# BenWibking/amrVolumeRenderer

Hardware: AMD Instinct MI355X
Metric: Mray-samples/s (2048x2048 render of 512^3-base 3-level AMR) (higher is better)
Workload: dtype f32 march / f64 cell fetch+transform; 1 GPU; config4_amr3_512: 176 boxes of 128^3 (2.95 GB f64), 3 AMR levels, field=smooth, 2048x2048, antialiasing=1, box_transparency=0.97, default jet map, 1 view(s); ownership=level_pairs, runs_total=1, frame_driver=C++ (avr_renderer: 3 HIP streams), march_workgroups_per_cu=0, classification=every frame, samples_per_frame=759136367, camera=static (the frame plan is made once)

## Files before the change

amrvolumerenderer_amd/csrc/avr_kernels.hip:

```cpp
#include <hip/hip_runtime.h>

#include <algorithm>
#include <cmath>
#include <cstdint>
#include <type_traits>

#include "avr_internal.h"
#include "avr_device.h"

namespace avr {

namespace {

constexpr int kBlockThreads = 256;
#ifndef AVR_MARCH_GROUP
#define AVR_MARCH_GROUP 8
#endif

#define AVR_INF __builtin_huge_valf()

struct Layer5 {
  float r, g, b, a, d;
};

// ... 13 lines not shown
  const float t = 1.0f - front.a;
  Layer5 out;
  out.r = front.r + back.r * t;
  out.g = front.g + back.g * t;
  out.b = front.b + back.b * t;
  out.a = front.a + back.a * t;
  out.d = (bottom.d < top.d) ? bottom.d : top.d;
  return out;
}

struct Ray {
  float ox, oy, oz;
  float dx, dy, dz;
};

__device__ __forceinline__ Ray make_ray(int px, int py, const FrameConsts& fc) {
  const float ndc_x = (static_cast<float>(px) + 0.5f) * fc.inv_width * 2.0f - 1.0f;
  const float ndc_y = (static_cast<float>(py) + 0.5f) * fc.inv_height * 2.0f - 1.0f;
  const float plane_x = ndc_x * fc.tan_half_fov * fc.aspect;
  const float plane_y = ndc_y * fc.tan_half_fov;
  Ray ray;
  ray.dx = fc.fwd[0] + plane_x * fc.right[0] + plane_y * fc.up[0];
  ray.dy = fc.fwd[1] + plane_x * fc.right[1] + plane_y * fc.up[1];
  ray.dz = fc.fwd[2] + plane_x * fc.right[2] + plane_y * fc.up[2];
  const float len_sq = ray.dx * ray.dx + ray.dy * ray.dy + ray.dz * ray.dz;
  const float len = (len_sq > 0.0f) ? (1.0f / (1.0f / sqrtf(len_sq))) : 0.0f;
  if (len > 0.0f) {
    const float inv = 1.0f / len;
    ray.dx *= inv;
    ray.dy *= inv;
    ray.dz *= inv;
  }
  ray.ox = fc.eye[0];
  ray.oy = fc.eye[1];
  ray.oz = fc.eye[2];
  return ray;
}

__device__ __forceinline__ void slab_axis(float origin, float direction, float inv_dir,
                                          float min_val, float max_val, float& tmin,
                                          float& tmax) {
  if (fabsf(direction) < 1e-8f) {
    if (origin < min_val || origin > max_val) {
      tmin = AVR_INF;
      tmax = -AVR_INF;
    }
    return;
  }
  float t1 = (min_val - origin) * inv_dir;
  float t2 = (max_val - origin) * inv_dir;
  if (t1 > t2) {
    const float tmp = t1;
    t1 = t2;
    t2 = tmp;
  }
  tmin = (tmin > t1) ? tmin : t1;
  tmax = (tmax < t2) ? tmax : t2;
}

__device__ __forceinline__ uint32_t bricklet_offset(int i, int j, int k, uint32_t y_pitch,
                                                    uint32_t x_pitch) {
  const uint32_t ui = static_cast<uint32_t>(i), uj = static_cast<uint32_t>(j),
                 uk = static_cast<uint32_t>(k);
  uint32_t offset;
  asm("v_lshl_add_u32 %0, %1, 3, %2" : "=v"(offset) : "v"(uj), "v"(ui));
  asm("v_lshl_add_u32 %0, %1, 5, %0" : "+v"(offset) : "v"(uk));
  asm("v_mad_u32_u24 %0, %1, %2, %0" : "+v"(offset) : "v"(uj >> 2), "s"(y_pitch));
  asm("v_mad_u32_u24 %0, %1, %2, %0" : "+v"(offset) : "v"(ui >> 3), "s"(x_pitch));
  return offset;
}

template <bool LINEAR>
__device__ __forceinline__ uint32_t cell_address(int i, int j, int k, uint32_t y_pitch,
                                                 uint32_t x_pitch) {
  if constexpr (LINEAR) {
    return (static_cast<uint32_t>(i) + static_cast<uint32_t>(j) * y_pitch +
            static_cast<uint32_t>(k) * x_pitch) << 3;
  } else {
    return bricklet_offset(i, j, k, y_pitch, x_pitch);
  }
}

typedef float float_pair __attribute__((ext_vector_type(2)));

template <int MODE, bool CLAMP, bool STATS, bool LINEAR = false>
__device__ __forceinline__ uint32_t offset_from_quotients(const BoxDev& box, uint32_t row_pitch,
                                                          uint32_t plane_pitch, float qx, float qy,
                                                          float qz, float fx, float fy, float fz,
                                                          unsigned& near_hits) {
  int i = static_cast<int>(qx);
  int j = static_cast<int>(qy);
  int k = static_cast<int>(qz);
  if (CLAMP) {
    i = (i > box.nx - 1) ? box.nx - 1 : i;
    j = (j > box.ny - 1) ? box.ny - 1 : j;
    k = (k > box.nz - 1) ? box.nz - 1 : k;
  }
  if (MODE == kReciprocal) {
    const float ex = fabsf(qx - rintf(qx));
    const float ey = fabsf(qy - rintf(qy));
    const float ez = fabsf(qz - rintf(qz));
    if (fminf(fminf(ex, ey), ez) <= box.near_tol) {
      if (STATS) ++near_hits;
      int ei = static_cast<int>(floorf(fx / box.dx));
      int ej = static_cast<int>(floorf(fy / box.dy));
      int ek = static_cast<int>(floorf(fz / box.dz));
      i = (ei < 0) ? 0 : ((ei >= box.nx) ? box.nx - 1 : ei);
      j = (ej < 0) ? 0 : ((ej >= box.ny) ? box.ny - 1 : ej);
      k = (ek < 0) ? 0 : ((ek >= box.nz) ? box.nz - 1 : ek);
    }
  }
  return cell_address<LINEAR>(i, j, k, row_pitch, plane_pitch);
}

template <int MODE, bool STATS, bool LINEAR = false>
__device__ __forceinline__ uint32_t cell_offset(const BoxDev& box, uint32_t row_pitch,
                                                uint32_t plane_pitch, float fx, float fy,
                                                float fz, unsigned& near_hits) {
  if (MODE == kExactDivide) {
    int ei = static_cast<int>(floorf(fx / box.dx));
    int ej = static_cast<int>(floorf(fy / box.dy));
    int ek = static_cast<int>(floorf(fz / box.dz));
    ei = (ei < 0) ? 0 : ((ei >= box.nx) ? box.nx - 1 : ei);
    ej = (ej < 0) ? 0 : ((ej >= box.ny) ? box.ny - 1 : ej);
    ek = (ek < 0) ? 0 : ((ek >= box.nz) ? box.nz - 1 : ek);
    return cell_address<LINEAR>(ei, ej, ek, row_pitch, plane_pitch);
  }
  return offset_from_quotients<MODE, true, STATS, LINEAR>(box, row_pitch, plane_pitch, fx * box.inv_dx,
                                                  fy * box.inv_dy, fz * box.inv_dz, fx, fy, fz,
                                                  near_hits);
}

struct ColumnSum {
  double sum;
  unsigned count;
};
template <FrameKind KIND> struct MarchOf { using Result = Layer5; using RayArg = const Ray&; };
template <> struct MarchOf<FrameKind::kMaxIntensity> { using Result = int; using RayArg = const Ray; };
template <> struct MarchOf<FrameKind::kProjection> { using Result = ColumnSum; using RayArg = const Ray; };

template <bool STATS, int MODE, FrameKind KIND = FrameKind::kVolume>
__device__ __forceinline__ typename MarchOf<KIND>::Result
march_box(const BoxDev& box, const FrameConsts& fc,
                                            const uint8_t* __restrict__ classified,
                                            const float4* __restrict__ table,
                                            typename MarchOf<KIND>::RayArg ray,
                                            float tmin, float tmax, unsigned& fetches,
                                            unsigned& near_hits) {
  constexpr bool is_max = KIND == FrameKind::kMaxIntensity, is_sum = KIND == FrameKind::kProjection;
  const float min_x = box.minc[0], min_y = box.minc[1], min_z = box.minc[2];
  const float max_x = box.maxc[0], max_y = box.maxc[1], max_z = box.maxc[2];
  const float step = box.sample_dist;
  const uint8_t __attribute__((address_space(1)))* cells =
      (const uint8_t __attribute__((address_space(1)))*)(classified + box.cls_offset);
  const uint32_t bricks_z = static_cast<uint32_t>(box.nz + kBrickZ - 1) >> 2;
  const uint32_t bricks_y = static_cast<uint32_t>(box.ny + kBrickY - 1) >> 2;
  const uint32_t row_pitch = is_sum ? static_cast<uint32_t>(box.jstride)
                                 : bricks_z * kBrickBytes - 32u;
  const uint32_t plane_pitch = is_sum ? static_cast<uint32_t>(box.kstride)
                                   : bricks_y * bricks_z * kBrickBytes - 8u;
  [[maybe_unused]] const uint8_t __attribute__((address_space(1)))* values =
      (const uint8_t __attribute__((address_space(1)))*)(box.cells);

  float distance = tmin + box.mesh_eps;
  if (distance < 0.0f) distance = box.mesh_eps;

  float acc_r = 0.0f, acc_g = 0.0f, acc_b = 0.0f, acc_a = 0.0f;
  [[maybe_unused]] int best = -1;
  [[maybe_unused]] double sum = 0.0;
  [[maybe_unused]] unsigned count = 0u;

#define AVR_INSIDE(x, y, z) \
  (!((x) < min_x || (x) > max_x || (y) < min_y || (y) > max_y || (z) < min_z || (z) > max_z))
#define AVR_VALUE(offset) \
  (*reinterpret_cast<const double __attribute__((address_space(1)))*>(values + (offset)))
#define AVR_ADD(value)                                  \
  do {                                                  \
    const bool finite_ = __builtin_isfinite(value);     \
    sum += finite_ ? (value) : 0.0;                     \
    count += finite_ ? 1u : 0u;                         \
  } while (0)
#define AVR_ACCUMULATE(sample)                          \
  do {                                                  \
    const float alpha_ = (sample).w * (1.0f - acc_a);   \
    acc_r += (sample).x * alpha_;                       \
    acc_g += (sample).y * alpha_;                       \
    acc_b += (sample).z * alpha_;                       \
    acc_a += alpha_;                                    \
  } while (0)

  const float safe_end = tmax - step;
  bool interior = false;
  if (distance < safe_end) {
    const float ax = ray.ox + ray.dx * distance, ay = ray.oy + ray.dy * distance,
                az = ray.oz + ray.dz * distance;
    const float bx = ray.ox + ray.dx * safe_end, by = ray.oy + ray.dy * safe_end,
                bz = ray.oz + ray.dz * safe_end;
    interior = AVR_INSIDE(ax, ay, az) && AVR_INSIDE(bx, by, bz);
    if (MODE != kExactDivide) {
      const int ia = static_cast<int>((ax - min_x) * box.inv_dx), ib = static_cast<int>((bx - min_x) * box.inv_dx);
      const int ja = static_cast<int>((ay - min_y) * box.inv_dy), jb = static_cast<int>((by - min_y) * box.inv_dy);
      const int ka = static_cast<int>((az - min_z) * box.inv_dz), kb = static_cast<int>((bz - min_z) * box.inv_dz);
      interior = interior && ia < box.nx && ib < box.nx && ja < box.ny && jb < box.ny &&
                 ka < box.nz && kb < box.nz;
    }
  }
  if (interior) {
    const float inv_x = box.inv_dx, inv_y = box.inv_dy, inv_z = box.inv_dz;
    const float_pair ix2 = {inv_x, inv_x}, iy2 = {inv_y, inv_y}, iz2 = {inv_z, inv_z};
    float_pair nx2 = {box.nmin_inv[0], box.nmin_inv[0]}, ny2 = {box.nmin_inv[1], box.nmin_inv[1]},
               nz2 = {box.nmin_inv[2], box.nmin_inv[2]};
    if (MODE == kPow2Multiply) asm volatile("" : "+v"(nx2), "+v"(ny2), "+v"(nz2));
#if AVR_MARCH_GROUP > 4
    if (MODE == kPow2Multiply || MODE == kReciprocal) {
      constexpr int kDeep = AVR_MARCH_GROUP;
      static_assert(kDeep % 2 == 0, "the positions are computed two at a time");
      for (;;) {
        float d[kDeep];
        d[0] = distance;
#pragma unroll
        for (int i = 1; i < kDeep; ++i) d[i] = d[i - 1] + step;
        if (!(d[kDeep - 1] < safe_end)) break;
        uint32_t off[kDeep];
#pragma unroll
        for (int pair = 0; pair < kDeep / 2; ++pair) {
          const float_pair dd = {d[2 * pair], d[2 * pair + 1]};
          if (MODE == kPow2Multiply) {
            const float_pair qx = __builtin_elementwise_fma(ray.ox + ray.dx * dd, ix2, nx2);
            const float_pair qy = __builtin_elementwise_fma(ray.oy + ray.dy * dd, iy2, ny2);
            const float_pair qz = __builtin_elementwise_fma(ray.oz + ray.dz * dd, iz2, nz2);
            off[2 * pair] = cell_address<is_sum>(static_cast<int>(qx.x), static_cast<int>(qy.x),
                                            static_cast<int>(qz.x), row_pitch, plane_pitch);
            off[2 * pair + 1] = cell_address<is_sum>(static_cast<int>(qx.y), static_cast<int>(qy.y),
                                                static_cast<int>(qz.y), row_pitch, plane_pitch);
          } else {
            const float_pair fx = (ray.ox + ray.dx * dd) - min_x;
            const float_pair fy = (ray.oy + ray.dy * dd) - min_y;
            const float_pair fz = (ray.oz + ray.dz * dd) - min_z;
            const float_pair qx = fx * inv_x, qy = fy * inv_y, qz = fz * inv_z;
            off[2 * pair] = offset_from_quotients<MODE, false, STATS, is_sum>(
                box, row_pitch, plane_pitch, qx.x, qy.x, qz.x, fx.x, fy.x, fz.x, near_hits);
            off[2 * pair + 1] = offset_from_quotients<MODE, false, STATS, is_sum>(
                box, row_pitch, plane_pitch, qx.y, qy.y, qz.y, fx.y, fy.y, fz.y, near_hits);
          }
        }
        if constexpr (is_sum) {
          double v[kDeep];
#pragma unroll
          for (int i = 0; i < kDeep; ++i) v[i] = AVR_VALUE(off[i]);
#pragma unroll
          for (int i = 0; i < kDeep; ++i) AVR_ADD(v[i]);
          distance = d[kDeep - 1] + step;
          if (STATS) fetches += static_cast<unsigned>(kDeep);
          continue;
        }
        int idx[kDeep];
#pragma unroll
        for (int i = 0; i < kDeep; ++i) idx[i] = cells[off[i]];
        if constexpr (is_max) {
#pragma unroll
          for (int i = 0; i < kDeep; ++i) best = (idx[i] > best) ? idx[i] : best;
          distance = d[kDeep - 1] + step;
          if (STATS) fetches += static_cast<unsigned>(kDeep);
          continue;
        }
        float4 sample[kDeep];
#pragma unroll
        for (int i = 0; i < kDeep; ++i) sample[i] = table[idx[i]];
        float_pair rg = {acc_r, acc_g}, ba = {acc_b, acc_a};
#pragma unroll
        for (int i = 0; i < kDeep; ++i) {
          const float w_ = sample[i].w * (1.0f - ba.y);
          const float_pair color_ = {sample[i].x, sample[i].y};
          const float_pair zw_ = {sample[i].z * w_, w_};
          float_pair weighted_;
          asm("v_pk_mul_f32 %0, %1, %2 op_sel:[0,1] op_sel_hi:[1,1]"
              : "=v"(weighted_)
              : "v"(color_), "v"(zw_));
          ba = ba + zw_;
          rg = rg + weighted_;
          asm volatile("" : "+v"(rg));
        }
        if (__builtin_amdgcn_ballot_w64(ba.y >= 1.0f) == 0) {
          acc_r = rg.x;
          acc_g = rg.y;
          acc_b = ba.x;
          acc_a = ba.y;
          distance = d[kDeep - 1] + step;
          if (STATS) fetches += static_cast<unsigned>(kDeep);
        } else {
          unsigned taken = 0u;
          float next = distance;
#pragma unroll
          for (int i = 0; i < kDeep; ++i) {
            const bool running_ = acc_a < 1.0f;
            const float alpha_ = sample[i].w * (1.0f - acc_a);
            const float r_ = acc_r + sample[i].x * alpha_;
            const float g_ = acc_g + sample[i].y * alpha_;
            const float b_ = acc_b + sample[i].z * alpha_;
            const float a_ = acc_a + alpha_;
            acc_r = running_ ? r_ : acc_r;
            acc_g = running_ ? g_ : acc_g;
            acc_b = running_ ? b_ : acc_b;
            acc_a = running_ ? a_ : acc_a;
            next = running_ ? (d[i] + step) : next;
            taken += running_ ? 1u : 0u;
          }
          distance = next;
          if (STATS) fetches += taken;
          if (!(acc_a < 1.0f)) break;
        }
      }
    }
#endif
    for (;;) {
      const float d1 = distance;
      const float d2 = d1 + step;
      const float d3 = d2 + step;
      const float d4 = d3 + step;
      if (!(d4 < safe_end)) break;
      uint32_t off1, off2, off3, off4;
      if (MODE == kExactDivide) {
        off1 = cell_offset<MODE, STATS, is_sum>(box, row_pitch, plane_pitch,
                                        (ray.ox + ray.dx * d1) - min_x,
                                        (ray.oy + ray.dy * d1) - min_y,
                                        (ray.oz + ray.dz * d1) - min_z, near_hits);
        off2 = cell_offset<MODE, STATS, is_sum>(box, row_pitch, plane_pitch,
                                        (ray.ox + ray.dx * d2) - min_x,
                                        (ray.oy + ray.dy * d2) - min_y,
                                        (ray.oz + ray.dz * d2) - min_z, near_hits);
        off3 = cell_offset<MODE, STATS, is_sum>(box, row_pitch, plane_pitch,
                                        (ray.ox + ray.dx * d3) - min_x,
                                        (ray.oy + ray.dy * d3) - min_y,
                                        (ray.oz + ray.dz * d3) - min_z, near_hits);
        off4 = cell_offset<MODE, STATS, is_sum>(box, row_pitch, plane_pitch,
                                        (ray.ox + ray.dx * d4) - min_x,
                                        (ray.oy + ray.dy * d4) - min_y,
                                        (ray.oz + ray.dz * d4) - min_z, near_hits);
      } else if (MODE == kPow2Multiply) {
        const float_pair d12 = {d1, d2}, d34 = {d3, d4};
        const float_pair qx12 = __builtin_elementwise_fma(ray.ox + ray.dx * d12, ix2, nx2);
        const float_pair qy12 = __builtin_elementwise_fma(ray.oy + ray.dy * d12, iy2, ny2);
        const float_pair qz12 = __builtin_elementwise_fma(ray.oz + ray.dz * d12, iz2, nz2);
        const float_pair qx34 = __builtin_elementwise_fma(ray.ox + ray.dx * d34, ix2, nx2);
        const float_pair qy34 = __builtin_elementwise_fma(ray.oy + ray.dy * d34, iy2, ny2);
        const float_pair qz34 = __builtin_elementwise_fma(ray.oz + ray.dz * d34, iz2, nz2);
        off1 = cell_address<is_sum>(static_cast<int>(qx12.x), static_cast<int>(qy12.x),
                               static_cast<int>(qz12.x), row_pitch, plane_pitch);
        off2 = cell_address<is_sum>(static_cast<int>(qx12.y), static_cast<int>(qy12.y),
                               static_cast<int>(qz12.y), row_pitch, plane_pitch);
        off3 = cell_address<is_sum>(static_cast<int>(qx34.x), static_cast<int>(qy34.x),
                               static_cast<int>(qz34.x), row_pitch, plane_pitch);
        off4 = cell_address<is_sum>(static_cast<int>(qx34.y), static_cast<int>(qy34.y),
                               static_cast<int>(qz34.y), row_pitch, plane_pitch);
      } else {
        const float_pair d12 = {d1, d2}, d34 = {d3, d4};
        const float_pair fx12 = (ray.ox + ray.dx * d12) - min_x, fx34 = (ray.ox + ray.dx * d34) - min_x;
        const float_pair fy12 = (ray.oy + ray.dy * d12) - min_y, fy34 = (ray.oy + ray.dy * d34) - min_y;
        const float_pair fz12 = (ray.oz + ray.dz * d12) - min_z, fz34 = (ray.oz + ray.dz * d34) - min_z;
        const float_pair qx12 = fx12 * inv_x, qx34 = fx34 * inv_x;
        const float_pair qy12 = fy12 * inv_y, qy34 = fy34 * inv_y;
        const float_pair qz12 = fz12 * inv_z, qz34 = fz34 * inv_z;
        off1 = offset_from_quotients<MODE, false, STATS, is_sum>(box, row_pitch, plane_pitch, qx12.x,
                                                         qy12.x, qz12.x, fx12.x, fy12.x, fz12.x,
                                                         near_hits);
        off2 = offset_from_quotients<MODE, false, STATS, is_sum>(box, row_pitch, plane_pitch, qx12.y,
                                                         qy12.y, qz12.y, fx12.y, fy12.y, fz12.y,
                                                         near_hits);
        off3 = offset_from_quotients<MODE, false, STATS, is_sum>(box, row_pitch, plane_pitch, qx34.x,
                                                         qy34.x, qz34.x, fx34.x, fy34.x, fz34.x,
                                                         near_hits);
        off4 = offset_from_quotients<MODE, false, STATS, is_sum>(box, row_pitch, plane_pitch, qx34.y,
                                                         qy34.y, qz34.y, fx34.y, fy34.y, fz34.y,
                                                         near_hits);
      }
      if constexpr (is_sum) {
        const double v1 = AVR_VALUE(off1);
        const double v2 = AVR_VALUE(off2);
        const double v3 = AVR_VALUE(off3);
        const double v4 = AVR_VALUE(off4);
        AVR_ADD(v1);
        AVR_ADD(v2);
        AVR_ADD(v3);
        AVR_ADD(v4);
        distance = d4 + step;
        if (STATS) fetches += 4u;
        continue;
      }
      const int idx1 = cells[off1];
      const int idx2 = cells[off2];
      const int idx3 = cells[off3];
      const int idx4 = cells[off4];
      if constexpr (is_max) {
        const int m12 = (idx1 > idx2) ? idx1 : idx2;
        const int m34 = (idx3 > idx4) ? idx3 : idx4;
        const int m = (m12 > m34) ? m12 : m34;
        best = (m > best) ? m : best;
        distance = d4 + step;
        if (STATS) fetches += 4u;
        continue;
      }
      const float4 s1 = table[idx1];
      const float4 s2 = table[idx2];
      const float4 s3 = table[idx3];
      const float4 s4 = table[idx4];
      float_pair rg = {acc_r, acc_g}, ba = {acc_b, acc_a};
#define AVR_STEP(sample)                                                          \
      {                                                                           \
        const float w_ = (sample).w * (1.0f - ba.y);                              \
        const float_pair color_ = {(sample).x, (sample).y};                       \
        const float_pair zw_ = {(sample).z * w_, w_};                             \
        float_pair weighted_;                                                     \
        asm("v_pk_mul_f32 %0, %1, %2 op_sel:[0,1] op_sel_hi:[1,1]"                \
            : "=v"(weighted_)                                                     \
            : "v"(color_), "v"(zw_));                                             \
        ba = ba + zw_;                                                            \
        rg = rg + weighted_;                                                      \
        asm volatile("" : "+v"(rg));                                              \
      }
      AVR_STEP(s1)
      AVR_STEP(s2)
      AVR_STEP(s3)
      AVR_STEP(s4)
#undef AVR_STEP
      if (__builtin_amdgcn_ballot_w64(ba.y >= 1.0f) == 0) {
        acc_r = rg.x;
        acc_g = rg.y;
        acc_b = ba.x;
        acc_a = ba.y;
// ... 11 lines not shown
          const float g_ = acc_g + (sample).y * alpha_;       \
          const float b_ = acc_b + (sample).z * alpha_;       \
          const float a_ = acc_a + alpha_;                    \
          acc_r = running_ ? r_ : acc_r;                      \
          acc_g = running_ ? g_ : acc_g;                      \
          acc_b = running_ ? b_ : acc_b;                      \
          acc_a = running_ ? a_ : acc_a;                      \
          next = running_ ? (following) : next;               \
          taken += running_ ? 1u : 0u;                        \
        }
        AVR_ACCUMULATE_IF_RUNNING(s2, d3)
        AVR_ACCUMULATE_IF_RUNNING(s3, d4)
        AVR_ACCUMULATE_IF_RUNNING(s4, d4 + step)
#undef AVR_ACCUMULATE_IF_RUNNING
        distance = next;
        if (STATS) fetches += taken;
        if (!(acc_a < 1.0f)) break;
      }
    }
  }

  float pos_x = ray.ox + ray.dx * distance;
  float pos_y = ray.oy + ray.dy * distance;
  float pos_z = ray.oz + ray.dz * distance;

  while (distance < tmax && (is_max || is_sum || acc_a < 1.0f)) {
    if (AVR_INSIDE(pos_x, pos_y, pos_z)) {
      const uint32_t offset = cell_offset<MODE, STATS, is_sum>(
          box, row_pitch, plane_pitch, pos_x - min_x, pos_y - min_y, pos_z - min_z, near_hits);
      if constexpr (is_sum) {
        const double v = AVR_VALUE(offset);
        if (STATS) ++fetches;
        AVR_ADD(v);
      } else {
      const int idx = cells[offset];
      if (STATS) ++fetches;
      if constexpr (is_max) {
        best = (idx > best) ? idx : best;
      } else {
        const float4 sample = table[idx];
        AVR_ACCUMULATE(sample);
      }
      }
    }
    distance += step;
    pos_x = ray.ox + ray.dx * distance;
    pos_y = ray.oy + ray.dy * distance;
    pos_z = ray.oz + ray.dz * distance;
  }
#undef AVR_INSIDE
#undef AVR_ACCUMULATE
#undef AVR_VALUE
#undef AVR_ADD

  if constexpr (is_sum) {
    return ColumnSum{sum, count};
  } else if constexpr (is_max) {
    return best;
  } else {
    acc_r = (acc_r > 1.0f) ? 1.0f : acc_r;
    acc_g = (acc_g > 1.0f) ? 1.0f : acc_g;
    acc_b = (acc_b > 1.0f) ? 1.0f : acc_b;
    acc_a = (acc_a > 1.0f) ? 1.0f : acc_a;
    Layer5 out;
    out.r = (acc_r < 0.0f) ? 0.0f : acc_r;
    out.g = (acc_g < 0.0f) ? 0.0f : acc_g;
    out.b = (acc_b < 0.0f) ? 0.0f : acc_b;
    out.a = (acc_a < 0.0f) ? 0.0f : acc_a;

    float depth = AVR_INF;
    if (acc_a > 0.0f) {
      const float ex = ray.ox + ray.dx * tmin;
      const float ey = ray.oy + ray.dy * tmin;
      const float ez = ray.oz + ray.dz * tmin;
      depth = (ex - fc.eye[0]) * fc.fwd[0] + (ey - fc.eye[1]) * fc.fwd[1] +
              (ez - fc.eye[2]) * fc.fwd[2];
    }
    if (!__builtin_isfinite(depth) || out.a <= 0.0f) depth = AVR_INF;
    out.d = depth;
    return out;
  }
}

template <bool STATS, int ONLY_MODE, bool SPEC, FrameKind KIND = FrameKind::kVolume>
__device__ __forceinline__ void
render_runs_body(
    const FrameConsts& fc, const BoxDev* __restrict__ boxes,
    const uint8_t* __restrict__ classified, const float* __restrict__ tables,
    const int n_tables, const int32_t* __restrict__ order, const int4* __restrict__ order_rects,
    const int32_t* __restrict__ run_end,
    const int n_runs, const int n_pieces, const RunRectDev* __restrict__ run_rects,
    const RunBlockDev* __restrict__ run_blocks, const RunSpanDev* __restrict__ run_spans,
    const int band_shift,
    const int tiles_x, const int tiles_y,
    const MarchItemDev* __restrict__ items, float* __restrict__ out,
    unsigned long long* samples_out, unsigned long long* counters,
    const int pos_begin, const int pos_end, const int resume,
    uint8_t* __restrict__ visible_out,
    const MarchSpecDev* __restrict__ spec) {
  constexpr bool is_max = KIND == FrameKind::kMaxIntensity, is_sum = KIND == FrameKind::kProjection;
  extern __shared__ float4 lds_tables[];
  if (SPEC && spec != nullptr) {
    const uint32_t* const gate = spec->gate;
    if (gate != nullptr) {
      if (*gate == 0) return;
      const uint8_t* const dirty = spec->dirty_blocks;
      if (dirty != nullptr && dirty[blockIdx.x] == 0) return;
    }
  }

  const unsigned b = blockIdx.x;
  const unsigned xcd = b % kXcds;
  const unsigned within = b / kXcds;
  const MarchItemDev item = items[(within / kSuperTileTiles) * kXcds + xcd];
  if (item.slot == kNoMarchItem) return;
  const unsigned seq = item.slot * kSuperTileTiles + (within % kSuperTileTiles);
  const int tile_x = static_cast<int>(compact_bits(seq));
  const int tile_y = static_cast<int>(compact_bits(seq >> 1));
  if (tile_x >= tiles_x || tile_y >= tiles_y) return;
  const int run = static_cast<int>(item.run);
  const RunRectDev rect = run_rects[run];
  if (rect.x1 < tile_x * kTile || rect.x0 > tile_x * kTile + kTile - 1 ||
      rect.y1 < tile_y * kTile || rect.y0 > tile_y * kTile + kTile - 1) {
    return;
  }

  if constexpr (!is_sum) {
  {
    const float4* src = reinterpret_cast<const float4*>(tables);
    const int total = n_tables * kTableSize;
    for (int e = threadIdx.x; e < total; e += kBlockThreads) lds_tables[e] = src[e];
  }
  __syncthreads();
  }

  const int wave = __builtin_amdgcn_readfirstlane(static_cast<int>(threadIdx.x) >> 6);
  const int lane = static_cast<int>(threadIdx.x) & 63;
  constexpr int kWaveW = 8, kWaveH = 8;
  const int wave_x0 = tile_x * kTile + (wave & 1) * 8;
  const int wave_y0 = tile_y * kTile + (wave >> 1) * 8;
  const int px = wave_x0 + (lane & 3) + ((lane >> 2) & 4);
  const int py = wave_y0 + ((lane >> 2) & 3) + ((lane >> 3) & 4);
  const bool live = (px < fc.width) && (py < fc.height);
  const int64_t n_pixels = static_cast<int64_t>(fc.width) * fc.height;
  const int64_t p = static_cast<int64_t>(py) * fc.width + px;

  const Ray ray = make_ray(px, py, fc);
  const float inv_dx = 1.0f / ray.dx;
  const float inv_dy = 1.0f / ray.dy;
  const float inv_dz = 1.0f / ray.dz;

  unsigned fetches = 0;
  unsigned near_hits = 0, mode_fetches[3] = {0u, 0u, 0u};
  {
    auto layer_pixel = [&]() -> float* {
      if (!(live && px >= rect.x0 && px <= rect.x1 && py >= rect.y0 && py <= rect.y1)) return nullptr;
      int64_t piece;
      int row = py;
      if (band_shift >= 0) {
        const unsigned band = static_cast<unsigned>(py) >> band_shift;
        const unsigned cycle = band / static_cast<unsigned>(n_pieces);
        piece = band - cycle * static_cast<unsigned>(n_pieces);
        row = static_cast<int>((cycle << band_shift) + (static_cast<unsigned>(py) & ((1u << band_shift) - 1u)));
      } else {
        const int64_t piece_size = n_pixels / n_pieces;
        piece = (piece_size > 0) ? (p / piece_size) : (n_pieces - 1);
        if (piece > n_pieces - 1) piece = n_pieces - 1;
      }
      const RunBlockDev block = run_blocks[static_cast<int64_t>(run) * n_pieces + piece];
      if (block.span_base >= 0) {
        const RunSpanDev span = run_spans[block.span_base + (row - block.first_row)];
        if (px < static_cast<int>(span.x0) || px > static_cast<int>(span.x1)) return nullptr;
        return out + block.offset + span.rel + static_cast<int64_t>(px - static_cast<int>(span.x0)) * 5;
      }
      return out + block.offset +
             (static_cast<int64_t>(row - block.first_row) * (rect.x1 - rect.x0 + 1) + (px - rect.x0)) * 5;
    };
    const int run_begin = (run > 0) ? run_end[run - 1] : 0;
    const int end = (run_end[run] < pos_end) ? run_end[run] : pos_end;
    Layer5 acc = {0.0f, 0.0f, 0.0f, 0.0f, AVR_INF};
    [[maybe_unused]] int acc_index = -1;
    [[maybe_unused]] double acc_column = 0.0, acc_length = 0.0;
    if (!is_max && !is_sum && resume != 0) {
      const float* src = layer_pixel();
      if (src != nullptr) {
        acc.r = src[0];
        acc.g = src[1];
        acc.b = src[2];
        acc.a = src[3];
        acc.d = src[4];
      }
    }
    for (int base = (run_begin > pos_begin) ? run_begin : pos_begin; base < end; base += 64) {
      bool candidate = false;
      if (base + lane < end) {
        const int4 r = order_rects[base + lane];
        candidate = !(r.z < wave_x0 || r.x > wave_x0 + (kWaveW - 1) || r.w < wave_y0 ||
                      r.y > wave_y0 + (kWaveH - 1));
      }
      unsigned long long pending = __builtin_amdgcn_ballot_w64(candidate);
      unsigned long long unclassified = 0;
      if (SPEC && spec != nullptr) {
        const uint8_t* const covered = spec->classified;
        if (covered != nullptr) {
          const bool missing = candidate && covered[base + lane] == 0;
          unclassified = __builtin_amdgcn_ballot_w64(missing);
        }
      }
      while (pending != 0) {
      const int bit = __builtin_ctzll(pending);
      const int position = base + bit;
      pending &= pending - 1;
      const BoxDev& box = boxes[order[position]];
      float tmin = -AVR_INF;
      float tmax = AVR_INF;
      slab_axis(ray.ox, ray.dx, inv_dx, box.minc[0], box.maxc[0], tmin, tmax);
      slab_axis(ray.oy, ray.dy, inv_dy, box.minc[1], box.maxc[1], tmin, tmax);
      slab_axis(ray.oz, ray.dz, inv_dz, box.minc[2], box.maxc[2], tmin, tmax);
      bool hit = live && (tmax >= tmin);
      if constexpr (is_max) {
        if (!__builtin_amdgcn_ballot_w64(hit)) continue;
        if (hit) {
          int m;
          if (ONLY_MODE == kPow2Multiply) {
            m = march_box<STATS, kPow2Multiply, KIND>(box, fc, classified, nullptr, ray, tmin, tmax,
                                                      fetches, near_hits);
          } else if (ONLY_MODE == kReciprocal) {
            m = march_box<STATS, kReciprocal, KIND>(box, fc, classified, nullptr, ray, tmin, tmax,
                                                    fetches, near_hits);
          } else if (box.index_mode == kPow2Multiply) {
            m = march_box<STATS, kPow2Multiply, KIND>(box, fc, classified, nullptr, ray, tmin, tmax,
                                                      fetches, near_hits);
          } else if (box.index_mode == kReciprocal) {
            m = march_box<STATS, kReciprocal, KIND>(box, fc, classified, nullptr, ray, tmin, tmax,
                                                    fetches, near_hits);
          } else {
            m = march_box<STATS, kExactDivide, KIND>(box, fc, classified, nullptr, ray, tmin, tmax,
                                                     fetches, near_hits);
          }
          acc_index = (m > acc_index) ? m : acc_index;
        }
        continue;
      }
      if constexpr (is_sum) {
        if (!__builtin_amdgcn_ballot_w64(hit)) continue;
        if (hit) {
          ColumnSum c;
          if (ONLY_MODE == kPow2Multiply) {
            c = march_box<STATS, kPow2Multiply, KIND>(box, fc, nullptr, nullptr, ray, tmin,
                                                             tmax, fetches, near_hits);
          } else if (ONLY_MODE == kReciprocal) {
            c = march_box<STATS, kReciprocal, KIND>(box, fc, nullptr, nullptr, ray, tmin, tmax,
                                                           fetches, near_hits);
          } else if (box.index_mode == kPow2Multiply) {
            c = march_box<STATS, kPow2Multiply, KIND>(box, fc, nullptr, nullptr, ray, tmin,
                                                             tmax, fetches, near_hits);
          } else if (box.index_mode == kReciprocal) {
            c = march_box<STATS, kReciprocal, KIND>(box, fc, nullptr, nullptr, ray, tmin, tmax,
                                                           fetches, near_hits);
          } else {
            c = march_box<STATS, kExactDivide, KIND>(box, fc, nullptr, nullptr, ray, tmin,
                                                            tmax, fetches, near_hits);
          }
          const double step = static_cast<double>(box.sample_dist);
          acc_column += step * c.sum;
          acc_length += step * static_cast<double>(c.count);
        }
        continue;
      }
      if (hit && acc.a == 1.0f) {
        const float ex = ray.ox + ray.dx * tmin;
        const float ey = ray.oy + ray.dy * tmin;
        const float ez = ray.oz + ray.dz * tmin;
        const float entry_depth = (ex - fc.eye[0]) * fc.fwd[0] + (ey - fc.eye[1]) * fc.fwd[1] +
                                  (ez - fc.eye[2]) * fc.fwd[2];
        if (acc.d <= entry_depth) hit = false;
      }
      if (!__builtin_amdgcn_ballot_w64(hit)) continue;
      if (SPEC && spec != nullptr) {
        if ((unclassified >> bit) & 1ull) {
          if (lane == 0) {
// ... 54 lines not shown
        bool visible = live && (tmax >= tmin);
        if (visible && !open && acc.a == 1.0f) {
          const float ex = ray.ox + ray.dx * tmin;
          const float ey = ray.oy + ray.dy * tmin;
          const float ez = ray.oz + ray.dz * tmin;
          const float entry_depth = (ex - fc.eye[0]) * fc.fwd[0] + (ey - fc.eye[1]) * fc.fwd[1] +
                                    (ez - fc.eye[2]) * fc.fwd[2];
          if (acc.d <= entry_depth) visible = false;
        }
        open = open || visible;
        if (__builtin_amdgcn_ballot_w64(visible) != 0 && lane == 0) visible_out[position] = 1;
      }
    }
    if constexpr (is_max) {
      if (acc_index >= 0) {
        const float4 c = lds_tables[acc_index];
        acc = {c.x, c.y, c.z, 1.0f, static_cast<float>(acc_index)};
      }
    }
    if constexpr (is_sum) {
      if (acc_length > 0.0) {
        const uint64_t column = static_cast<uint64_t>(__double_as_longlong(acc_column));
        const uint64_t length = static_cast<uint64_t>(__double_as_longlong(acc_length));
        acc = {__uint_as_float(static_cast<uint32_t>(column)),
               __uint_as_float(static_cast<uint32_t>(column >> 32)),
               __uint_as_float(static_cast<uint32_t>(length)), 1.0f,
               __uint_as_float(static_cast<uint32_t>(length >> 32))};
      }
    }
    {
      float* const dst = layer_pixel();
      if (STATS && counters != nullptr && dst == nullptr && acc.a != 0.0f && live && px >= rect.x0 &&
          px <= rect.x1 && py >= rect.y0 && py <= rect.y1) {
        atomicAdd(counters + 4, 1ull);
      }
      if (dst != nullptr) {
        dst[0] = acc.r;
        dst[1] = acc.g;
        dst[2] = acc.b;
        dst[3] = acc.a;
        dst[4] = acc.d;
      }
    }
  }

  if (STATS && samples_out != nullptr) {
    unsigned long long total = fetches;
    for (int offset = 32; offset > 0; offset >>= 1) {
      total += __shfl_down(total, offset, 64);
    }
    if (lane == 0 && total != 0) atomicAdd(samples_out, total);
    if (counters != nullptr) {
      const unsigned values[4] = {near_hits, mode_fetches[kExactDivide], mode_fetches[kReciprocal],
                                  mode_fetches[kPow2Multiply]};
#pragma unroll
      for (int c = 0; c < 4; ++c) {
        unsigned long long sum = values[c];
        for (int offset = 32; offset > 0; offset >>= 1) sum += __shfl_down(sum, offset, 64);
        if (lane == 0 && sum != 0) atomicAdd(counters + c, sum);
      }
    }
  }
}

#define AVR_MARCH_PARAMETERS                                                                       \
    const FrameConsts fc, const BoxDev* __restrict__ boxes, const uint8_t* __restrict__ classified, \
    const float* __restrict__ tables, const int n_tables, const int32_t* __restrict__ order,       \
    const int4* __restrict__ order_rects, const int32_t* __restrict__ run_end, const int n_runs,   \
    const int n_pieces, const RunRectDev* __restrict__ run_rects,                                  \
    const RunBlockDev* __restrict__ run_blocks, const RunSpanDev* __restrict__ run_spans,          \
    const int band_shift, const int tiles_x, const int tiles_y,                                    \
    const MarchItemDev* __restrict__ items, float* __restrict__ out,                               \
    unsigned long long* samples_out, unsigned long long* counters, const int pos_begin,            \
    const int pos_end, const int resume, uint8_t* __restrict__ visible_out,                        \
    const MarchSpecDev* __restrict__ spec
#define AVR_MARCH_ARGUMENTS                                                                        \
    fc, boxes, classified, tables, n_tables, order, order_rects, run_end, n_runs, n_pieces,        \
    run_rects, run_blocks, run_spans, band_shift, tiles_x, tiles_y, items, out, samples_out,       \
    counters, pos_begin, pos_end, resume, visible_out, spec

constexpr int kMarchMinWorkgroups =
    AVR_MARCH_GROUP >= 16 ? 3 : AVR_MARCH_GROUP >= 8 ? 4 : AVR_MARCH_GROUP >= 6 ? 5 : 6;

template <bool STATS, int ONLY_MODE, bool SPEC = false>
__global__ __launch_bounds__(kBlockThreads, kMarchMinWorkgroups) void render_runs_kernel(AVR_MARCH_PARAMETERS) {
  render_runs_body<STATS, ONLY_MODE, SPEC>(AVR_MARCH_ARGUMENTS);
}

template <int ONLY_MODE>
__global__ __launch_bounds__(kBlockThreads, kMarchMinWorkgroups) void render_runs_repair_kernel(AVR_MARCH_PARAMETERS) {
  render_runs_body<false, ONLY_MODE, true>(AVR_MARCH_ARGUMENTS);
}
template <bool STATS, int ONLY_MODE>
__global__ __launch_bounds__(kBlockThreads, kMarchMinWorkgroups) void render_runs_max_kernel(AVR_MARCH_PARAMETERS) {
  render_runs_body<STATS, ONLY_MODE, false, FrameKind::kMaxIntensity>(AVR_MARCH_ARGUMENTS);
}
template <bool STATS, int ONLY_MODE>
__global__ __launch_bounds__(kBlockThreads, kMarchMinWorkgroups) void render_runs_sum_kernel(AVR_MARCH_PARAMETERS) {
  render_runs_body<STATS, ONLY_MODE, false, FrameKind::kProjection>(AVR_MARCH_ARGUMENTS);
}
#undef AVR_MARCH_PARAMETERS
#undef AVR_MARCH_ARGUMENTS

__global__ void upload_kernel(const uint4* __restrict__ src, uint4* __restrict__ dst, size_t n) {
  const size_t stride = static_cast<size_t>(gridDim.x) * blockDim.x;
  for (size_t i = static_cast<size_t>(blockIdx.x) * blockDim.x + threadIdx.x; i < n; i += stride) {
    dst[i] = src[i];
  }
}

__global__ void stall_kernel(unsigned long long ticks, unsigned int max_iterations) {
  const unsigned long long begin = wall_clock64();
  for (unsigned int i = 0; i < max_iterations; ++i) {
    if (wall_clock64() - begin >= ticks) break;
    __builtin_amdgcn_s_sleep(127);
  }
}

constexpr int kStagedStride = 34;
constexpr int kRawBufferFlags = 0x00020000;
constexpr int kStreamingLoad = 2;

template <bool SIMPLE>
__device__ __forceinline__ void classify_tile(
    const FrameConsts& fc, const BoxDev* __restrict__ boxes,
    const uint32_t* __restrict__ tile_begin, const int n_boxes, uint8_t* __restrict__ classified,
    const int stream_stores,
    const int32_t* __restrict__ box_list,
    const uint8_t* __restrict__ visible, const uint32_t tile, uint32_t* const staged) {
  int lo = 0, hi = n_boxes;
  while (hi - lo > 1) {
    const int mid = (lo + hi) >> 1;
    if (tile_begin[mid] <= tile) {
      lo = mid;
    } else {
      hi = mid;
    }
  }
  if (visible != nullptr && visible[lo] == 0) return;
  const BoxDev& box = boxes[box_list != nullptr ? box_list[lo] : lo];
  const int nx = box.nx, ny = box.ny, nz = box.nz;
  const int bricks_x = (nx + kBrickX - 1) >> 3;
  const int bricks_y = (ny + kBrickY - 1) >> 2;
  const int chunks = (nx + kClassifyChunk - 1) / kClassifyChunk;
  uint32_t local = tile - tile_begin[lo];
  const int chunk = static_cast<int>(local % static_cast<uint32_t>(chunks));
  local /= static_cast<uint32_t>(chunks);
  const int bj = static_cast<int>(local % static_cast<uint32_t>(bricks_y));
  const int bk = static_cast<int>(local / static_cast<uint32_t>(bricks_y));

  const double __attribute__((address_space(1)))* cells =
      (const double __attribute__((address_space(1)))*)box.cells;
  const uint32_t jstride = static_cast<uint32_t>(box.jstride);
  const uint32_t kstride = static_cast<uint32_t>(box.kstride);
  const int t = static_cast<int>(threadIdx.x);
  const bool paired = ((reinterpret_cast<uintptr_t>(box.cells) & 15u) == 0) &&
                      ((jstride & 1u) == 0) && ((kstride & 1u) == 0) && jstride < (1u << 27);
  typedef double double2_t __attribute__((ext_vector_type(2)));
  const bool whole_tile = SIMPLE && paired && (chunk + 1) * kClassifyChunk <= nx &&
                          (bj + 1) * kBrickY <= ny && (bk + 1) * kBrickZ <= nz;
  if (whole_tile) {
    const int jj = t >> 6;
    const int xi = (t & 63) * 2;
    const uint32_t lane_bytes = (static_cast<uint32_t>(chunk * kClassifyChunk + xi) +
                                 static_cast<uint32_t>(bj * kBrickY + jj) * jstride) * 8u;
    const __amdgpu_buffer_rsrc_t resource = __builtin_amdgcn_make_buffer_rsrc(
        const_cast<double*>(box.cells), 0, 0x7fffffff, kRawBufferFlags);
    double2_t raw[4];
#pragma unroll
    for (int pass = 0; pass < 4; ++pass) {
      const uint32_t plane_bytes = static_cast<uint32_t>(bk * kBrickZ + pass) * kstride * 8u;
      raw[pass] = __builtin_bit_cast(
          double2_t, __builtin_amdgcn_raw_buffer_load_b128(resource, lane_bytes, plane_bytes, kStreamingLoad));
    }
    char* const staged_at = reinterpret_cast<char*>(staged) + (xi >> 3) * (kStagedStride * 4) + jj * 8 + (xi & 7);
#pragma unroll
    for (int pass = 0; pass < 4; ++pass) {
      const double a = raw[pass].x, b = raw[pass].y;
      float sa = __builtin_amdgcn_fmed3f(static_cast<float>((a - fc.norm_min) * fc.inv_norm_span), 0.0f, 1.0f) * 255.0f;
      float sb = __builtin_amdgcn_fmed3f(static_cast<float>((b - fc.norm_min) * fc.inv_norm_span), 0.0f, 1.0f) * 255.0f;
      const bool odd = !__builtin_isfinite(a) || !__builtin_isfinite(b);
      if (__builtin_expect(__builtin_amdgcn_ballot_w64(odd) != 0, 0)) {
// ... 663 lines not shown
    }
    return check_launch("classify_gated_kernel");
  }
  if (simple) {
    hipLaunchKernelGGL(classify_kernel<true>, dim3(L.n_classify_tiles), dim3(kBlockThreads), pad,
                       stream, L.consts, L.boxes_dev, L.tile_begin_dev, n_listed, L.classified,
                       L.classify_stream_stores, L.box_list_dev, L.visible_in);
  } else {
    hipLaunchKernelGGL(classify_kernel<false>, dim3(L.n_classify_tiles), dim3(kBlockThreads), pad,
                       stream, L.consts, L.boxes_dev, L.tile_begin_dev, n_listed, L.classified,
                       L.classify_stream_stores, L.box_list_dev, L.visible_in);
  }
  return check_launch("classify_kernel");
}

template <typename F>
void with_march_variant(bool stats, int only_mode, F&& f) {
  const auto with_mode = [&](auto stats_c) {
    if (only_mode == kPow2Multiply) {
      f(stats_c, std::integral_constant<int, kPow2Multiply>{});
    } else if (only_mode == kReciprocal) {
      f(stats_c, std::integral_constant<int, kReciprocal>{});
    } else {
      f(stats_c, std::integral_constant<int, -1>{});
    }
  };
  if (stats) with_mode(std::true_type{}); else with_mode(std::false_type{});
}

int launch_march(const RenderLaunch& L, void* stream_v) {
  hipStream_t stream = static_cast<hipStream_t>(stream_v);
  const int tiles_x = (L.consts.width + kTile - 1) / kTile;
  const int tiles_y = (L.consts.height + kTile - 1) / kTile;
  const unsigned blocks = L.n_items * kSuperTileTiles;
  if (blocks == 0) return AVR_OK;
  size_t lds_bytes = L.kind == FrameKind::kProjection
                         ? 0
                         : static_cast<size_t>(L.n_tables) * kTableSize * sizeof(float4);
  if (L.workgroups_per_cu > 0) {
    const size_t share = (150 * 1024 / static_cast<size_t>(L.workgroups_per_cu)) & ~size_t{1023};
    lds_bytes = std::max(lds_bytes, share);
  }
  const bool stats = L.samples_out != nullptr;
  int band_shift = -1;
  if (L.pieces.layout == kPiecesRowBands) {
    band_shift = 0;
    while ((1 << band_shift) < L.pieces.band_rows) ++band_shift;
    if ((1 << band_shift) != L.pieces.band_rows) {
      set_error("render_runs_kernel: band_rows must be a power of two");
      return AVR_ERR_INVALID_ARGUMENT;
    }
  }
  const auto launch = [&](auto kernel) {
    hipLaunchKernelGGL(kernel, dim3(blocks), dim3(kBlockThreads), lds_bytes, stream, L.consts,
                       L.boxes_dev, L.classified, L.tables_dev, L.n_tables, L.order_dev,
                       reinterpret_cast<const int4*>(L.order_rects_dev), L.run_end_dev, L.n_runs,
                       L.n_pieces, L.run_rects_dev, L.run_blocks_dev, L.run_spans_dev, band_shift,
                       tiles_x, tiles_y, L.items_dev, L.out_layers, L.samples_out, L.counters,
                       L.pos_begin, (L.pos_end < 0 ? L.n_order : L.pos_end), L.resume,
                       L.visible_out, L.spec_dev);
  };
  if (L.spec_dev != nullptr) {
    if (stats) {
      set_error("render_runs_kernel: a speculative frame cannot count samples");
      return AVR_ERR_INVALID_ARGUMENT;
    }
    with_march_variant(false, L.only_mode, [&](auto, auto only) {
      launch(L.spec_is_repair ? render_runs_repair_kernel<only()> : render_runs_kernel<false, only(), true>);
    });
    return check_launch("render_runs_kernel (speculative)");
  }
  if (L.kind == FrameKind::kMaxIntensity) {
    with_march_variant(stats, L.only_mode, [&](auto stats_c, auto only) {
      launch(render_runs_max_kernel<stats_c(), only()>);
    });
    return check_launch("render_runs_max_kernel");
  }
  if (L.kind == FrameKind::kProjection) {
    with_march_variant(stats, L.only_mode, [&](auto stats_c, auto only) {
      launch(render_runs_sum_kernel<stats_c(), only()>);
    });
    return check_launch("render_runs_sum_kernel");
  }
  with_march_variant(stats, L.only_mode, [&](auto stats_c, auto only) {
    launch(render_runs_kernel<stats_c(), only()>);
  });
  return check_launch("render_runs_kernel");
}

int launch_blend(int kind, const void* top, const void* bottom, void* out, int64_t n,
                 void* stream_v) {
  hipStream_t stream = static_cast<hipStream_t>(stream_v);
  if (n <= 0) return AVR_OK;
  const int grid = grid_for(n, 256);
  if (kind == 0) {
    hipLaunchKernelGGL(blend_depthsort_kernel, dim3(grid), dim3(256), 0, stream,
                       static_cast<const float*>(top), static_cast<const float*>(bottom),
                       static_cast<float*>(out), n);
  } else if (kind == 1) {
    hipLaunchKernelGGL(blend_rgba_f32_kernel, dim3(grid), dim3(256), 0, stream,
                       static_cast<const float4*>(top), static_cast<const float4*>(bottom),
                       static_cast<float4*>(out), n);
  } else {
    hipLaunchKernelGGL(blend_rgba_u8_kernel, dim3(grid), dim3(256), 0, stream,
                       static_cast<const uint32_t*>(top), static_cast<const uint32_t*>(bottom),
                       static_cast<uint32_t*>(out), n);
  }
  return check_launch("blend kernel");
}

int launch_blend_regions(int kind, const void* top, int64_t tb, int64_t te, const void* bottom,
                         int64_t bb, int64_t be, void* out, void* stream_v) {
  hipStream_t stream = static_cast<hipStream_t>(stream_v);
  const int64_t ob = tb < bb ? tb : bb;
  const int64_t oe = te > be ? te : be;
  const int64_t n = oe - ob;
  if (n <= 0) return AVR_OK;
  const int grid = grid_for(n, 256);
  if (kind == 0) {
    hipLaunchKernelGGL(blend_regions_kernel<0>, dim3(grid), dim3(256), 0, stream, top, tb, te,
                       bottom, bb, be, out);
  } else if (kind == 1) {
    hipLaunchKernelGGL(blend_regions_kernel<1>, dim3(grid), dim3(256), 0, stream, top, tb, te,
                       bottom, bb, be, out);
  } else {
    hipLaunchKernelGGL(blend_regions_kernel<2>, dim3(grid), dim3(256), 0, stream, top, tb, te,
                       bottom, bb, be, out);
  }
  return check_launch("blend_regions_kernel");
}

int launch_encode_u8(const float* rgba, uint32_t* out, int64_t n, void* stream_v) {
  if (n <= 0) return AVR_OK;
  hipLaunchKernelGGL(encode_u8_kernel, dim3(grid_for(n, 256)), dim3(256), 0,
                     static_cast<hipStream_t>(stream_v), reinterpret_cast<const float4*>(rgba), out,
                     n);
  return check_launch("encode_u8_kernel");
}

int launch_decode_u8(const uint32_t* in, float* rgba, int64_t n, void* stream_v) {
  if (n <= 0) return AVR_OK;
  hipLaunchKernelGGL(decode_u8_kernel, dim3(grid_for(n, 256)), dim3(256), 0,
                     static_cast<hipStream_t>(stream_v), in, reinterpret_cast<float4*>(rgba), n);
  return check_launch("decode_u8_kernel");
}

constexpr int64_t kFoldWorkgroups = 2048;

int launch_fold_plan(const FoldLaunch& L, void* stream_v) {
  const int64_t n = L.piece_end - L.piece_begin;
  if (n <= 0) return AVR_OK;
  const int first_row = static_cast<int>(L.piece_begin / L.width);
  const int last_row = static_cast<int>((L.piece_end - 1) / L.width);
  const int chunks_per_row = (L.width + 255) / 256;
  const int64_t blocks = static_cast<int64_t>(last_row - first_row + 1) * chunks_per_row;
  if (blocks > 0x7fffffffLL) {
    set_error("fold_plan_kernel: image too large");
    return AVR_ERR_INVALID_ARGUMENT;
  }
  const int64_t grid = std::min<int64_t>(blocks, L.max_workgroups > 0 ? L.max_workgroups : kFoldWorkgroups);
  const bool own = L.own_end > L.own_begin;
  const auto launch = [&](const auto& out, const char* what) {
    constexpr FrameKind kind = std::decay_t<decltype(out)>::kKind;
    const auto kernel = own ? fold_plan_kernel<true, kind> : fold_plan_kernel<false, kind>;
    hipLaunchKernelGGL(kernel, dim3(static_cast<unsigned>(grid)), dim3(256), 0,
                       static_cast<hipStream_t>(stream_v), L.width, L.piece_begin, L.piece_end,
                       L.n_runs, L.run_rects_dev, L.run_blocks_dev, L.run_spans_dev, L.recv, out.first,
                       out.second, first_row, chunks_per_row, L.pieces, L.piece, L.own_begin,
// ... 107 lines not shown
```

Measured before the change: 855,000 Mray-samples/s.

## Trim march kernel register pressure and specialize volume march on launch window

Several micro-optimizations to the ray-march kernel. The pow2 quotient now uses a packed FMA whose scale and offset come from one SGPR pair. The saturated-tail step distance is accumulated incrementally, and the 4-sample tail loop is skipped once a ray is already opaque. Pixel-index and run-rect loads are moved late into the layer lambda, and the wave overlap test uses shifted tile coordinates. A new WINDOW template parameter compiles out the window begin, end, resume and visible-output handling for plain volume frames, aiming to cut VGPR/SGPR usage and instruction count at the cost of extra kernel variants.

```diff
diff --git a/amrvolumerenderer_amd/csrc/avr_kernels.hip b/amrvolumerenderer_amd/csrc/avr_kernels.hip
--- a/amrvolumerenderer_amd/csrc/avr_kernels.hip
+++ b/amrvolumerenderer_amd/csrc/avr_kernels.hip
@@ -119,6 +119,14 @@
 }
 
 typedef float float_pair __attribute__((ext_vector_type(2)));
+
+__device__ __forceinline__ float_pair fused_quotient(float_pair pos, float_pair inv_and_nmin) {
+  float_pair q;
+  asm("v_pk_fma_f32 %0, %1, %2, %2 op_sel:[0,0,1] op_sel_hi:[1,0,1]"
+      : "=v"(q)
+      : "v"(pos), "s"(inv_and_nmin));
+  return q;
+}
 
 template <int MODE, bool CLAMP, bool STATS, bool LINEAR = false>
 __device__ __forceinline__ uint32_t offset_from_quotients(const BoxDev& box, uint32_t row_pitch,
@@ -244,10 +252,8 @@
   }
   if (interior) {
     const float inv_x = box.inv_dx, inv_y = box.inv_dy, inv_z = box.inv_dz;
-    const float_pair ix2 = {inv_x, inv_x}, iy2 = {inv_y, inv_y}, iz2 = {inv_z, inv_z};
-    float_pair nx2 = {box.nmin_inv[0], box.nmin_inv[0]}, ny2 = {box.nmin_inv[1], box.nmin_inv[1]},
-               nz2 = {box.nmin_inv[2], box.nmin_inv[2]};
-    if (MODE == kPow2Multiply) asm volatile("" : "+v"(nx2), "+v"(ny2), "+v"(nz2));
+    const float_pair sx2 = {inv_x, box.nmin_inv[0]}, sy2 = {inv_y, box.nmin_inv[1]},
+                     sz2 = {inv_z, box.nmin_inv[2]};
 #if AVR_MARCH_GROUP > 4
     if (MODE == kPow2Multiply || MODE == kReciprocal) {
       constexpr int kDeep = AVR_MARCH_GROUP;
@@ -263,9 +269,9 @@
         for (int pair = 0; pair < kDeep / 2; ++pair) {
           const float_pair dd = {d[2 * pair], d[2 * pair + 1]};
           if (MODE == kPow2Multiply) {
-            const float_pair qx = __builtin_elementwise_fma(ray.ox + ray.dx * dd, ix2, nx2);
-            const float_pair qy = __builtin_elementwise_fma(ray.oy + ray.dy * dd, iy2, ny2);
-            const float_pair qz = __builtin_elementwise_fma(ray.oz + ray.dz * dd, iz2, nz2);
+            const float_pair qx = fused_quotient(ray.ox + ray.dx * dd, sx2);
+            const float_pair qy = fused_quotient(ray.oy + ray.dy * dd, sy2);
+            const float_pair qz = fused_quotient(ray.oz + ray.dz * dd, sz2);
             off[2 * pair] = cell_address<is_sum>(static_cast<int>(qx.x), static_cast<int>(qy.x),
                                             static_cast<int>(qz.x), row_pitch, plane_pitch);
             off[2 * pair + 1] = cell_address<is_sum>(static_cast<int>(qx.y), static_cast<int>(qy.y),
@@ -327,7 +333,8 @@
           if (STATS) fetches += static_cast<unsigned>(kDeep);
         } else {
           unsigned taken = 0u;
-          float next = distance;
+          float next = distance, following = distance;
+          asm volatile("" : "+v"(following));
 #pragma unroll
           for (int i = 0; i < kDeep; ++i) {
             const bool running_ = acc_a < 1.0f;
@@ -340,8 +347,10 @@
             acc_g = running_ ? g_ : acc_g;
             acc_b = running_ ? b_ : acc_b;
             acc_a = running_ ? a_ : acc_a;
-            next = running_ ? (d[i] + step) : next;
+            following += step;
+            next = running_ ? following : next;
             taken += running_ ? 1u : 0u;
+            asm volatile("" : "+v"(acc_r), "+v"(acc_g), "+v"(acc_b), "+v"(acc_a));
           }
           distance = next;
           if (STATS) fetches += taken;
@@ -350,7 +359,8 @@
       }
     }
 #endif
-    for (;;) {
+    const bool unsaturated = is_max || is_sum || acc_a < 1.0f;
+    for (; unsaturated;) {
       const float d1 = distance;
       const float d2 = d1 + step;
       const float d3 = d2 + step;
@@ -376,12 +386,12 @@
                                         (ray.oz + ray.dz * d4) - min_z, near_hits);
       } else if (MODE == kPow2Multiply) {
         const float_pair d12 = {d1, d2}, d34 = {d3, d4};
-        const float_pair qx12 = __builtin_elementwise_fma(ray.ox + ray.dx * d12, ix2, nx2);
-        const float_pair qy12 = __builtin_elementwise_fma(ray.oy + ray.dy * d12, iy2, ny2);
-        const float_pair qz12 = __builtin_elementwise_fma(ray.oz + ray.dz * d12, iz2, nz2);
-        const float_pair qx34 = __builtin_elementwise_fma(ray.ox + ray.dx * d34, ix2, nx2);
-        const float_pair qy34 = __builtin_elementwise_fma(ray.oy + ray.dy * d34, iy2, ny2);
-        const float_pair qz34 = __builtin_elementwise_fma(ray.oz + ray.dz * d34, iz2, nz2);
+        const float_pair qx12 = fused_quotient(ray.ox + ray.dx * d12, sx2);
+        const float_pair qy12 = fused_quotient(ray.oy + ray.dy * d12, sy2);
+        const float_pair qz12 = fused_quotient(ray.oz + ray.dz * d12, sz2);
+        const float_pair qx34 = fused_quotient(ray.ox + ray.dx * d34, sx2);
+        const float_pair qy34 = fused_quotient(ray.oy + ray.dy * d34, sy2);
+        const float_pair qz34 = fused_quotient(ray.oz + ray.dz * d34, sz2);
         off1 = cell_address<is_sum>(static_cast<int>(qx12.x), static_cast<int>(qy12.x),
                                static_cast<int>(qz12.x), row_pitch, plane_pitch);
         off2 = cell_address<is_sum>(static_cast<int>(qx12.y), static_cast<int>(qy12.y),
@@ -559,7 +569,7 @@
   }
 }
 
-template <bool STATS, int ONLY_MODE, bool SPEC, FrameKind KIND = FrameKind::kVolume>
+template <bool STATS, int ONLY_MODE, bool SPEC, bool WINDOW, FrameKind KIND = FrameKind::kVolume>
 __device__ __forceinline__ void
 render_runs_body(
     const FrameConsts& fc, const BoxDev* __restrict__ boxes,
@@ -572,11 +582,14 @@
     const int tiles_x, const int tiles_y,
     const MarchItemDev* __restrict__ items, float* __restrict__ out,
     unsigned long long* samples_out, unsigned long long* counters,
-    const int pos_begin, const int pos_end, const int resume,
-    uint8_t* __restrict__ visible_out,
+    const int window_begin, const int window_end, const int window_resume,
+    uint8_t* __restrict__ window_visible_out,
     const MarchSpecDev* __restrict__ spec) {
   constexpr bool is_max = KIND == FrameKind::kMaxIntensity, is_sum = KIND == FrameKind::kProjection;
   extern __shared__ float4 lds_tables[];
+  const int pos_begin = WINDOW ? window_begin : 0;
+  const int resume = WINDOW ? window_resume : 0;
+  uint8_t* const visible_out = WINDOW ? window_visible_out : nullptr;
   if (SPEC && spec != nullptr) {
     const uint32_t* const gate = spec->gate;
     if (gate != nullptr) {
@@ -619,8 +632,6 @@
   const int px = wave_x0 + (lane & 3) + ((lane >> 2) & 4);
   const int py = wave_y0 + ((lane >> 2) & 3) + ((lane >> 3) & 4);
   const bool live = (px < fc.width) && (py < fc.height);
-  const int64_t n_pixels = static_cast<int64_t>(fc.width) * fc.height;
-  const int64_t p = static_cast<int64_t>(py) * fc.width + px;
 
   const Ray ray = make_ray(px, py, fc);
   const float inv_dx = 1.0f / ray.dx;
@@ -630,7 +641,12 @@
   unsigned fetches = 0;
   unsigned near_hits = 0, mode_fetches[3] = {0u, 0u, 0u};
   {
+    const int whole_run = run;
     auto layer_pixel = [&]() -> float* {
+      const RunRectDev* late_rects = run_rects;
+      int run = whole_run;
+      asm volatile("" : "+s"(late_rects), "+s"(run));
+      const RunRectDev rect = late_rects[run];
       if (!(live && px >= rect.x0 && px <= rect.x1 && py >= rect.y0 && py <= rect.y1)) return nullptr;
       int64_t piece;
       int row = py;
@@ -640,6 +656,8 @@
         piece = band - cycle * static_cast<unsigned>(n_pieces);
         row = static_cast<int>((cycle << band_shift) + (static_cast<unsigned>(py) & ((1u << band_shift) - 1u)));
       } else {
+        const int64_t n_pixels = static_cast<int64_t>(fc.width) * fc.height;
+        const int64_t p = static_cast<int64_t>(py) * fc.width + px;
         const int64_t piece_size = n_pixels / n_pieces;
         piece = (piece_size > 0) ? (p / piece_size) : (n_pieces - 1);
         if (piece > n_pieces - 1) piece = n_pieces - 1;
@@ -654,7 +672,7 @@
              (static_cast<int64_t>(row - block.first_row) * (rect.x1 - rect.x0 + 1) + (px - rect.x0)) * 5;
     };
     const int run_begin = (run > 0) ? run_end[run - 1] : 0;
-    const int end = (run_end[run] < pos_end) ? run_end[run] : pos_end;
+    const int end = (!WINDOW || run_end[run] < window_end) ? run_end[run] : window_end;
     Layer5 acc = {0.0f, 0.0f, 0.0f, 0.0f, AVR_INF};
     [[maybe_unused]] int acc_index = -1;
     [[maybe_unused]] double acc_column = 0.0, acc_length = 0.0;
@@ -672,8 +690,13 @@
       bool candidate = false;
       if (base + lane < end) {
         const int4 r = order_rects[base + lane];
-        candidate = !(r.z < wave_x0 || r.x > wave_x0 + (kWaveW - 1) || r.w < wave_y0 ||
-                      r.y > wave_y0 + (kWaveH - 1));
+        static_assert(kWaveW == 8 && kWaveH == 8, "the shifts below");
+        int wave_col = px, wave_row = py;
+        asm volatile("" : "+v"(wave_col), "+v"(wave_row));
+        wave_col >>= 3;
+        wave_row >>= 3;
+        candidate = !((r.z >> 3) < wave_col || (r.x >> 3) > wave_col || (r.w >> 3) < wave_row ||
+                      (r.y >> 3) > wave_row);
       }
       unsigned long long pending = __builtin_amdgcn_ballot_w64(candidate);
       unsigned long long unclassified = 0;
@@ -894,22 +917,23 @@
 constexpr int kMarchMinWorkgroups =
     AVR_MARCH_GROUP >= 16 ? 3 : AVR_MARCH_GROUP >= 8 ? 4 : AVR_MARCH_GROUP >= 6 ? 5 : 6;
 
-template <bool STATS, int ONLY_MODE, bool SPEC = false>
+template <bool STATS, int ONLY_MODE, bool SPEC = false, bool WINDOW = SPEC>
 __global__ __launch_bounds__(kBlockThreads, kMarchMinWorkgroups) void render_runs_kernel(AVR_MARCH_PARAMETERS) {
-  render_runs_body<STATS, ONLY_MODE, SPEC>(AVR_MARCH_ARGUMENTS);
+  static_assert(WINDOW || !SPEC, "a speculative frame's march is compiled with the launch window");
+  render_runs_body<STATS, ONLY_MODE, SPEC, WINDOW>(AVR_MARCH_ARGUMENTS);
 }
 
 template <int ONLY_MODE>
 __global__ __launch_bounds__(kBlockThreads, kMarchMinWorkgroups) void render_runs_repair_kernel(AVR_MARCH_PARAMETERS) {
-  render_runs_body<false, ONLY_MODE, true>(AVR_MARCH_ARGUMENTS);
+  render_runs_body<false, ONLY_MODE, true, true>(AVR_MARCH_ARGUMENTS);
 }
 template <bool STATS, int ONLY_MODE>
 __global__ __launch_bounds__(kBlockThreads, kMarchMinWorkgroups) void render_runs_max_kernel(AVR_MARCH_PARAMETERS) {
-  render_runs_body<STATS, ONLY_MODE, false, FrameKind::kMaxIntensity>(AVR_MARCH_ARGUMENTS);
+  render_runs_body<STATS, ONLY_MODE, false, true, FrameKind::kMaxIntensity>(AVR_MARCH_ARGUMENTS);
 }
 template <bool STATS, int ONLY_MODE>
 __global__ __launch_bounds__(kBlockThreads, kMarchMinWorkgroups) void render_runs_sum_kernel(AVR_MARCH_PARAMETERS) {
-  render_runs_body<STATS, ONLY_MODE, false, FrameKind::kProjection>(AVR_MARCH_ARGUMENTS);
+  render_runs_body<STATS, ONLY_MODE, false, true, FrameKind::kProjection>(AVR_MARCH_ARGUMENTS);
 }
 #undef AVR_MARCH_PARAMETERS
 #undef AVR_MARCH_ARGUMENTS
@@ -1739,8 +1763,14 @@
     });
     return check_launch("render_runs_sum_kernel");
   }
+  const bool window = L.pos_begin != 0 || (L.pos_end >= 0 && L.pos_end < L.n_order) || L.resume != 0 ||
+                      L.visible_out != nullptr;
   with_march_variant(stats, L.only_mode, [&](auto stats_c, auto only) {
-    launch(render_runs_kernel<stats_c(), only()>);
+    if (window) {
+      launch(render_runs_kernel<stats_c(), only(), false, true>);
+    } else {
+      launch(render_runs_kernel<stats_c(), only(), false, false>);
+    }
   });
   return check_launch("render_runs_kernel");
 }
```

New measurement: 860,800 Mray-samples/s (median of 4 runs). Within noise of the previous version (+0.7%).
